# flash4242/Promptable-Counterfactual-GAN

Hardware: AMD Instinct MI355X
Metric: images/sec (G+D step) MNIST-28 cDCGAN bs512 @1/2/4/8 MI355X; % MFMA roofline (higher is better)
Workload: dtype f32

## Files before the change

include/pcgan_hip.h:

```cpp
#ifndef PCGAN_HIP_H
#define PCGAN_HIP_H

#include <stddef.h>
#include <stdint.h>

#ifdef __cplusplus
extern "C" {
#endif

typedef void* pcg_stream_t;

typedef enum pcg_status {
  PCG_OK = 0,
  PCG_ERR_INVALID = -1,
  PCG_ERR_WORKSPACE = -2,
  PCG_ERR_LAUNCH = -3,
  PCG_ERR_UNSUPPORTED = -4
} pcg_status;

typedef enum pcg_act {
  PCG_ACT_NONE = 0,
  PCG_ACT_RELU = 1,
  PCG_ACT_LRELU = 2,
  PCG_ACT_TANH = 3,
// ... 49 lines not shown
                         int64_t* num_batches_tracked, const float* gamma, const float* beta, float* coef_out ,
                         void* workspace, size_t workspace_bytes, pcg_stream_t stream);
int pcg_conv2d_dgrad_bn_xf(const pcg_conv_geom* g, const float* dy, const pcg_in_xform* xf, const float* w, const float* bias_x, float* dx,
                           float eps, float momentum, float* save_mean, float* save_invstd, float* running_mean, float* running_var,
                           int64_t* num_batches_tracked, const float* gamma, const float* beta, float* coef_out ,
                           void* workspace, size_t workspace_bytes, pcg_stream_t stream);
int pcg_conv2d_fwd_xf(const pcg_conv_geom* g, const float* x, const pcg_in_xform* xf, const float* w, const float* bias, int act,
                      float slope, float* y, void* workspace , size_t workspace_bytes, pcg_stream_t stream);
int pcg_conv2d_dgrad_xf(const pcg_conv_geom* g, const float* dy, const pcg_in_xform* xf, const float* w, const float* bias_x, int act,
                        float slope, float* dx, void* workspace , size_t workspace_bytes, pcg_stream_t stream);
int pcg_conv2d_wgrad_xf(const pcg_conv_geom* g, const float* x, const pcg_in_xform* xf_x, const float* dy, const pcg_in_xform* xf_dy,
                        float* dw, int accumulate, void* workspace, size_t workspace_bytes, pcg_stream_t stream);
int pcg_conv2d_dgrad_mask(const pcg_conv_geom* g, const float* dy, const float* w, const float* a_below, int act, float slope,
                          float* dx, void* workspace , size_t workspace_bytes, pcg_stream_t stream);
int32_t pcg_conv2d_dgrad_mask_thin_ok(const pcg_conv_geom* g);
int32_t pcg_conv2d_xf_thin_ok(const pcg_conv_geom* g);
int pcg_conv2d_fwd_add_mask(const pcg_conv_geom* g, const float* x, const float* w, const float* addend, const float* a_below, int act,
                            float slope, float* y, pcg_stream_t stream);
int pcg_conv2d_dgrad_add_mask(const pcg_conv_geom* g, const float* dy, const float* w, const float* addend, const float* a_below, int act,
                              float slope, float* dx, pcg_stream_t stream);
int pcg_conv2d_fwd_mask(const pcg_conv_geom* g, const float* x, const float* w, const float* a_below, int act, float slope,
                        float* y, void* workspace , size_t workspace_bytes, pcg_stream_t stream);
int pcg_conv2d_dgrad_bnbwd(const pcg_conv_geom* g, const float* dy, const float* w, const float* z_below, const float* mean,
                           const float* invstd, const float* gamma, const float* beta, int act, float slope, float* dx,
                           void* partial, size_t partial_bytes, pcg_stream_t stream);
int pcg_conv2d_fwd_bnbwd(const pcg_conv_geom* g, const float* x, const float* w, const float* z_below, const float* mean,
                         const float* invstd, const float* gamma, const float* beta, int act, float slope, float* y,
                         void* partial, size_t partial_bytes, pcg_stream_t stream);
int pcg_conv2d_dgrad_add(const pcg_conv_geom* g, const float* dy, const float* w, const float* addend, float* dx,
                         void* workspace , size_t workspace_bytes, pcg_stream_t stream);
// ... 440 lines not shown
```

promptable-counterfactual-gan_amd/_lib.py:

```python
import ctypes
import os

import torch

_HERE = os.path.dirname(os.path.abspath(__file__))
LIB_PATH = os.environ.get("PCG_LIB") or os.path.join(_HERE, "libpcgan_hip.so")

PCG_OK = 0
ACT_NONE, ACT_RELU, ACT_LRELU, ACT_TANH, ACT_SIGMOID = 0, 1, 2, 3, 4


class PcgError(RuntimeError):
    pass


class ConvGeom(ctypes.Structure):

    _fields_ = [(n, ctypes.c_int32) for n in ("B", "IH", "IW", "Cin", "OH", "OW", "Cout", "KH", "KW", "stride", "pad")]

    def key(self):
        return tuple(getattr(self, n) for n, _ in self._fields_)


_I, _P = ctypes.c_int32, ctypes.c_void_p
# ... 95 lines not shown
    "pcg_calib_mfma_workspace_bytes": (_sz, [_i32]),
    "pcg_calib_mfma": (_i, [_i32, _i32, _vp, _sz, _c.POINTER(_d), _c.POINTER(_c.c_uint64), _vp]),
    "pcg_calib_copy": (_i, [_vp, _vp, _i64, _vp]),
    "pcg_conv2d_fwd_workspace_bytes": (_sz, [_gp]),
    "pcg_conv2d_dgrad_workspace_bytes": (_sz, [_gp]),
    "pcg_conv2d_fwd": (_i, [_gp, _vp, _vp, _vp, _vp, _vp, _sz, _vp]),
    "pcg_conv2d_dgrad": (_i, [_gp, _vp, _vp, _vp, _vp, _vp, _sz, _vp]),
    "pcg_conv2d_fwd_act": (_i, [_gp, _vp, _vp, _vp, _i, _f, _vp, _vp, _sz, _vp]),
    "pcg_conv2d_dgrad_act": (_i, [_gp, _vp, _vp, _vp, _i, _f, _vp, _vp, _sz, _vp]),
    "pcg_conv2d_fwd_bn_workspace_bytes": (_sz, [_gp]),
    "pcg_conv2d_dgrad_bn_workspace_bytes": (_sz, [_gp]),
    "pcg_conv2d_fwd_bn": (_i, [_gp, _vp, _vp, _vp, _vp, _f, _f, _vp, _vp, _vp, _vp, _vp, _vp, _sz, _vp]),
    "pcg_conv2d_dgrad_bn": (_i, [_gp, _vp, _vp, _vp, _vp, _f, _f, _vp, _vp, _vp, _vp, _vp, _vp, _sz, _vp]),
    "pcg_conv2d_dgrad_mask": (_i, [_gp, _vp, _vp, _vp, _i, _f, _vp, _vp, _sz, _vp]),
    "pcg_conv2d_dgrad_mask_thin_ok": (_i32, [_gp]),
    "pcg_conv2d_xf_thin_ok": (_i32, [_gp]),
    "pcg_conv2d_fwd_add_mask": (_i, [_gp, _vp, _vp, _vp, _vp, _i, _f, _vp, _vp]),
    "pcg_conv2d_dgrad_add_mask": (_i, [_gp, _vp, _vp, _vp, _vp, _i, _f, _vp, _vp]),
    "pcg_conv2d_fwd_mask": (_i, [_gp, _vp, _vp, _vp, _i, _f, _vp, _vp, _sz, _vp]),
    "pcg_conv2d_dgrad_bnbwd": (_i, [_gp, _vp, _vp, _vp, _vp, _vp, _vp, _vp, _i, _f, _vp, _vp, _sz, _vp]),
    "pcg_conv2d_fwd_bnbwd": (_i, [_gp, _vp, _vp, _vp, _vp, _vp, _vp, _vp, _i, _f, _vp, _vp, _sz, _vp]),
    "pcg_conv2d_dgrad_add": (_i, [_gp, _vp, _vp, _vp, _vp, _vp, _sz, _vp]),
    "pcg_conv2d_fwd_bn_partial_rows": (_c.c_int32, [_gp]),
    "pcg_conv2d_dgrad_bn_partial_rows": (_c.c_int32, [_gp]),
    "pcg_bn_bwd_partial_workspace_bytes": (_sz, [_c.c_int32]),
    "pcg_bn_bwd_partial": (_i, [_vp, _vp, _i64, _c.c_int32, _vp, _vp, _vp, _vp, _c.c_int32, _vp, _vp, _vp, _i, _vp, _sz, _vp]),
    "pcg_conv2d_fwd_bn_xf": (_i, [_gp, _vp, _xp, _vp, _vp, _vp, _f, _f, _vp, _vp, _vp, _vp, _vp, _vp, _vp, _vp, _vp, _sz, _vp]),
    "pcg_conv2d_dgrad_bn_xf": (_i, [_gp, _vp, _xp, _vp, _vp, _vp, _f, _f, _vp, _vp, _vp, _vp, _vp, _vp, _vp, _vp, _vp, _sz, _vp]),
    "pcg_conv2d_fwd_xf": (_i, [_gp, _vp, _xp, _vp, _vp, _i, _f, _vp, _vp, _sz, _vp]),
    "pcg_conv2d_dgrad_xf": (_i, [_gp, _vp, _xp, _vp, _vp, _i, _f, _vp, _vp, _sz, _vp]),
# ... 177 lines not shown
```

promptable-counterfactual-gan_amd/csrc/conv_igemm.hip:

```cpp
#include <string.h>
#include <mutex>
#include "conv_loaders.h"
#include "thin_conv.h"

namespace pcg {
namespace {

__device__ __forceinline__ int wave_id() { return __builtin_amdgcn_readfirstlane((int)(threadIdx.x >> 6)); }

__device__ __forceinline__ void prio_entry(const ConvP& p) { if (p.edge_prio & 1) __builtin_amdgcn_s_setprio(3); }
__device__ __forceinline__ void prio_epilogue(const ConvP& p) { if (p.edge_prio & 2) __builtin_amdgcn_s_setprio(3); }

__device__ __forceinline__ int epi_group_off(const ConvP& p, int m_block) {
  return p.epi.group_rows > 0 ? __builtin_amdgcn_readfirstlane(m_block / p.epi.group_rows) * p.N : 0;
}

template <class Cfg, bool XF>
__global__ void __launch_bounds__(IG_THREADS, Cfg::MINW) conv_fwd_kernel(ConvP p) {
  extern __shared__ __attribute__((aligned(16))) float smem[];
  prio_entry(p);
  const uint32_t tile = xcd_remap(blockIdx.x, gridDim.x);
  const int mt = tile / p.tilesN, nt = tile % p.tilesN;
  const int m_block = mt * Cfg::BM, n_block = nt * Cfg::BN;
  const int kt_begin = blockIdx.y * p.ktiles_per_split;
// ... 59 lines not shown
    }
    DgradALoader<Cfg::BM, XF> la(p, f, m_block, tid);
    DgradBLoader<Cfg::BN> lb(p, f, n_block, tid);
    igemm_produce<Cfg>(la, lb, ktiles, smem, tid, ClockStamp{p.stamps, p.stamp_slots});
    return;
  }
  f32x16 acc[Cfg::TM][Cfg::TN];
  ClockStamp cs{p.stamps, p.stamp_slots};
  cs.phase(0);
  igemm_consume<Cfg, true, false>(ktiles, acc, smem, cs);
  prio_epilogue(p);
  igemm_store_tile<Cfg>(acc, smem, n_block, p.N, p.bias, [&](int row) -> float* {
    const int pix = rowpix[row];
    return pix >= 0 ? p.out + (size_t)pix * p.Cin + n_block : nullptr;
  }, p.stat_partial ? p.stat_partial + (size_t)(f.prow0 + mt * Cfg::WAVES_M) * 2 * p.N : nullptr, p.act, p.slope, &p.epi, epi_group_off(p, m_block));
  cs.phase(3);
}

struct SkPlan {
  int dp_tiles, sk_tiles, sk_blocks, ktiles;
  float* parts;
  int* arrivals;
};
struct SkSeg { int tile, kt_begin, nkt, nparts, first_block; };

__device__ __forceinline__ int sk_start(int g, const SkPlan& sk) {
  return __builtin_amdgcn_readfirstlane((int)((uint32_t)g * (uint32_t)(sk.sk_tiles * sk.ktiles) / (uint32_t)sk.sk_blocks));
}
__device__ __forceinline__ int sk_owner(int x, const SkPlan& sk) {
  return __builtin_amdgcn_readfirstlane((int)((((uint32_t)x + 1u) * (uint32_t)sk.sk_blocks - 1u) / (uint32_t)(sk.sk_tiles * sk.ktiles)));
// ... 981 lines not shown

extern "C" int32_t pcg_conv2d_xf_thin_ok(const pcg_conv_geom* g) { return check_geom(g) == PCG_OK && thin_conv_xf_ok(g) ? 1 : 0; }
extern "C" int32_t pcg_conv2d_dgrad_mask_thin_ok(const pcg_conv_geom* g) { return check_geom(g) == PCG_OK && thin_conv_dgrad_mask_ok(g) && g->Cin % 4 == 0 ? 1 : 0; }
extern "C" int pcg_conv2d_dgrad_mask(const pcg_conv_geom* g, const float* dy, const float* w, const float* a_below, int act, float slope,
                                     float* dx, void* workspace, size_t workspace_bytes, pcg_stream_t stream) {
  EpiAux e{};
  e.mode = EPI_MASK;
  if (int rc = check_geom(g)) return rc;
  if (pcg_conv2d_dgrad_mask_thin_ok(g)) {
    PCG_REQUIRE(dy && w && a_below && dx && (((uintptr_t)a_below | (uintptr_t)dx) & 15) == 0, "pcg_conv2d_dgrad_mask: null or misaligned tensor");
    PCG_REQUIRE(act == PCG_ACT_NONE || act == PCG_ACT_RELU || act == PCG_ACT_LRELU, "pcg_conv2d_dgrad_mask: activation %d is not none / ReLU / LeakyReLU", act);
    return thin_conv_dgrad_mask(g, dy, w, a_below, act, slope, dx, (hipStream_t)stream);
  }
  if (int rc = epi_common("pcg_conv2d_dgrad_mask", g, dx, a_below, act, slope, &e)) return rc;
  return conv2d_dgrad_impl(g, dy, w, nullptr, dx, nullptr, workspace, workspace_bytes, stream, PCG_ACT_NONE, 0.f, &e);
}
extern "C" int pcg_conv2d_fwd_mask(const pcg_conv_geom* g, const float* x, const float* w, const float* a_below, int act, float slope,
                                   float* y, void* workspace, size_t workspace_bytes, pcg_stream_t stream) {
  EpiAux e{};
  e.mode = EPI_MASK;
  if (int rc = check_geom(g)) return rc;
  if (int rc = epi_common("pcg_conv2d_fwd_mask", g, y, a_below, act, slope, &e)) return rc;
  return conv2d_fwd_impl(g, x, w, nullptr, y, nullptr, workspace, workspace_bytes, stream, PCG_ACT_NONE, 0.f, &e);
}

extern "C" int pcg_conv2d_dgrad_add(const pcg_conv_geom* g, const float* dy, const float* w, const float* addend, float* dx,
                                    void* workspace, size_t workspace_bytes, pcg_stream_t stream) {
  EpiAux e{};
  e.mode = EPI_ADD;
  if (int rc = check_geom(g)) return rc;
// ... 437 lines not shown
```

promptable-counterfactual-gan_amd/csrc/igemm_core.h:

```cpp
#pragma once
#include "pcg_common.h"

namespace pcg {

typedef float f32x16 __attribute__((ext_vector_type(16)));

typedef unsigned int u32x4 __attribute__((ext_vector_type(4)));
using rsrc_t = __amdgpu_buffer_rsrc_t;
constexpr uint32_t OOB_OFF = 0x80000000u;

__device__ __forceinline__ rsrc_t make_rsrc(const void* p, uint32_t bytes) {
  return __builtin_amdgcn_make_buffer_rsrc(const_cast<void*>(p), 0, bytes, 0x00020000);
}
__device__ __forceinline__ float4 buf_load4(rsrc_t r, uint32_t off) {
  const u32x4 v = __builtin_amdgcn_raw_buffer_load_b128(r, off, 0, 0);
  return make_float4(__uint_as_float(v.x), __uint_as_float(v.y), __uint_as_float(v.z), __uint_as_float(v.w));
}

constexpr int IG_LOADERS = 256;
constexpr int IG_THREADS = 512;
constexpr int IG_BK = 32;
#ifndef PCG_PREFETCH_DEPTH
#define PCG_PREFETCH_DEPTH 2
#endif
// ... 506 lines not shown
  }
  if (want_sums) {
#pragma unroll
    for (int off = Q; off < 64; off <<= 1) {
#pragma unroll
      for (int e = 0; e < 4; ++e) { s1[e] += __shfl_xor(s1[e], off); s2[e] += __shfl_xor(s2[e], off); }
    }
    if (r0 == 0 && nok) {
      double* pr = stat_row + (size_t)wm * 2 * N;
#pragma unroll
      for (int e = 0; e < 4; ++e) { pr[n + e] = s1[e]; pr[N + n + e] = s2[e]; }
    }
  }
}


}
```

promptable-counterfactual-gan_amd/csrc/thin_conv.h:

```cpp
#pragma once
#include "pcg_common.h"

namespace pcg {

inline bool thin_is_cin(const pcg_conv_geom* g) { return g->Cin <= 3; }
inline bool thin_is_cout(const pcg_conv_geom* g) { return g->Cout <= 3 && !thin_is_cin(g); }

struct ThinBnIn { const float* mean; const float* invstd; const float* gamma; const float* beta; int act; float slope; int groups; };
bool thin_conv_bnin_full_ok(const pcg_conv_geom* g, int groups);
int thin_conv_fwd(const pcg_conv_geom* g, const float* x, const float* w, const float* bias, float* y, void* ws,
                  size_t ws_bytes, hipStream_t s, int act = PCG_ACT_NONE, float slope = 0.f, const ThinBnIn* bnin = nullptr);
struct ThinXf { const float* scale; const float* shift; float neg; };
bool thin_conv_xf_ok(const pcg_conv_geom* g);
int thin_conv_dgrad(const pcg_conv_geom* g, const float* dy, const float* w, const float* bias_x, float* dx, void* ws,
                    size_t ws_bytes, hipStream_t s, int act = PCG_ACT_NONE, float slope = 0.f, const ThinXf* xf = nullptr);
size_t thin_conv_fwd_workspace_bytes(const pcg_conv_geom* g);
size_t thin_conv_dgrad_workspace_bytes(const pcg_conv_geom* g);
size_t thin_conv_wgrad_workspace_bytes(const pcg_conv_geom* g);
int thin_conv_wgrad(const pcg_conv_geom* g, const float* x, const float* dy, float* dw, int accumulate, void* ws,
                    size_t ws_bytes, hipStream_t s, const ThinXf* xf = nullptr, const ThinBnIn* bnin = nullptr);

bool thin_conv_fwd_bnbwd_ok(const pcg_conv_geom* g);
size_t thin_conv_fwd_bnbwd_workspace_bytes(const pcg_conv_geom* g);
int thin_conv_fwd_bnbwd(const pcg_conv_geom* g, const float* x, const float* w, const float* z, const float* mean, const float* invstd,
                        const float* gamma, const float* beta, int act, float slope, float* dz, float* dgamma, float* dbeta, int accumulate,
                        void* ws, size_t ws_bytes, hipStream_t s);

bool thin_conv_dgrad_mask_ok(const pcg_conv_geom* g);
int thin_conv_dgrad_mask(const pcg_conv_geom* g, const float* dy, const float* w, const float* a_below, int act, float slope, float* dx,
                         hipStream_t s);

bool thin_conv_dgrad_bnbwd_full_ok(const pcg_conv_geom* g, int groups);
size_t thin_conv_dgrad_bnbwd_full_workspace_bytes(const pcg_conv_geom* g, int groups);
int thin_conv_dgrad_bnbwd_full(const pcg_conv_geom* g, const float* dy, const float* w, const float* z, const float* mean, const float* invstd,
                               const float* gamma, const float* beta, int act, float slope, float* dz, float* dgamma, float* dbeta, int accumulate,
                               int groups, void* ws, size_t ws_bytes, hipStream_t s);

int launch_slab_reduce(const float* slab, float* dw, size_t n, size_t slab_stride, int nslabs, int accumulate, hipStream_t s, bool deferrable = false);

int slab_defer_begin(hipStream_t s);
int slab_defer_flush(hipStream_t s);
int slab_defer_pending();

}
```

promptable-counterfactual-gan_amd/csrc/thin_conv.hip:

```cpp
#include "thin_conv.h"
#include <cstdlib>

namespace pcg {
namespace {

struct ThinP {
  const float* thin;
  const float* wide;
  const float* w;
  const float* bias;
  float* out;
  int act; float slope;
  const float* xf_scale; const float* xf_shift; float xf_neg;
  const float* mask_src; float mask_neg;
  int B, TH, TW, Cs, WH, WW, C;
  int KH, KW, stride, pad, transposed;
  int wsS, wsT, wsC;
  int IH_, IW_;
  int QH, QW;
  int npix;
  FastDiv dIW, dIH, dCQ;
};

__device__ __forceinline__ bool tap_map(const ThinP& p, int ph, int pw, int kh, int kw, int& qh, int& qw) {
// ... 748 lines not shown
    }
    unsigned blocks = (unsigned)((n4 + 63) / 64);
    if (blocks > 4096) blocks = 4096;
    if (blocks == 0) blocks = 1;
    hipLaunchKernelGGL(slab_reduce4_kernel, dim3(blocks), dim3(64), 0, s, reinterpret_cast<const float4*>(slab),
                       reinterpret_cast<float4*>(dw), n4, slab_stride / 4, nslabs, accumulate);
  } else {
    unsigned blocks = (unsigned)((n + 255) / 256);
    if (blocks > 2048) blocks = 2048;
    if (blocks == 0) blocks = 1;
    hipLaunchKernelGGL(slab_reduce1_kernel, dim3(blocks), dim3(256), 0, s, slab, dw, n, slab_stride, nslabs, accumulate);
  }
  return launch_status("slab_reduce_kernel");
}

bool thin_conv_bnin_full_ok(const pcg_conv_geom* g, int groups) {
  if (!full_window(g) || groups < 1 || groups > 8 || g->B % groups || g->Cin % 4) return false;
  const int CQ = g->Cin / 4;
  return CQ <= 256 && 256 % CQ == 0 && (g->B / groups) % FULL_ROWS_DW == 0;
}
static FullXf full_xf_of(const pcg_conv_geom* g, const ThinBnIn* bi) {
  if (!bi || !bi->mean) return FullXf{nullptr, nullptr, nullptr, nullptr, 1.f, g->Cin, g->B};
  return FullXf{bi->mean, bi->invstd, bi->gamma, bi->beta, act_neg_of(bi->act, bi->slope), g->Cin, g->B / bi->groups};
}

int thin_conv_fwd(const pcg_conv_geom* g, const float* x, const float* w, const float* bias, float* y, void* ws,
                  size_t ws_bytes, hipStream_t s, int act, float slope, const ThinBnIn* bnin) {
  PCG_REQUIRE(!(bnin && bnin->mean) || (thin_conv_bnin_full_ok(g, bnin->groups) && (((uintptr_t)x | (uintptr_t)w) & 15) == 0),
              "thin conv forward: a BatchNorm input needs the full-window form (thin_conv_bnin_full_ok) and 16-byte aligned tensors");
  ThinP p{};
// ... 86 lines not shown
  if (cin_thin) { p.wide = dy; return launch_reduce(p, ws, ws_bytes, s); }
  p.thin = dy;
  const bool fuse = act_is_cheap(act);
  p.act = fuse ? act : PCG_ACT_NONE; p.slope = act_neg_of(p.act, slope);
  if (full_window(g) && bias_x == nullptr && (((uintptr_t)dx | (uintptr_t)w) & 15) == 0) {
    const int L4 = g->KH * g->KW * g->Cin / 4;
    hipLaunchKernelGGL(thin_full_outer_kernel, dim3((unsigned)((L4 + 255) / 256), (unsigned)((g->B + FULL_ROWS_DX - 1) / FULL_ROWS_DX)), dim3(256), 0, s, dy,
                       reinterpret_cast<const float4*>(w), reinterpret_cast<float4*>(dx), g->B, L4, p.slope);
    if (int e = launch_status("thin_full_outer_kernel")) return e;
    return fuse ? PCG_OK : pcg_act_fwd(dx, (int64_t)g->B * g->IH * g->IW * g->Cin, act, slope, dx, (pcg_stream_t)s);
  }
  if (int e = launch_expand(p, s)) return e;
  return fuse ? PCG_OK : pcg_act_fwd(dx, (int64_t)g->B * g->IH * g->IW * g->Cin, act, slope, dx, (pcg_stream_t)s);
}

bool thin_conv_dgrad_mask_ok(const pcg_conv_geom* g) {
  if (!thin_is_cout(g)) return false;
  ThinP p{};
  if (fill_common(p, g, false, false) != PCG_OK) return false;
  const bool k44 = p.KH == 4 && p.KW == 4, k33 = p.KH == 3 && p.KW == 3;
  RowsP rp{};
  size_t patch_bytes = 0;
  return (k44 || k33) && (k33 || p.Cs == 1) && lds_weight_bytes(p) <= 64 * 1024 && rows_plan(p, rp, &patch_bytes);
}
int thin_conv_dgrad_mask(const pcg_conv_geom* g, const float* dy, const float* w, const float* a_below, int act, float slope, float* dx,
                         hipStream_t s) {
  PCG_REQUIRE(thin_conv_dgrad_mask_ok(g), "thin grad-input with mask: only the row-block forms (k3 / k4 with a thin output)");
  ThinP p{};
  if (int e = fill_common(p, g, false, false)) return e;
  p.w = w; p.bias = nullptr; p.out = dx; p.thin = dy; p.act = PCG_ACT_NONE; p.slope = 0.f;
// ... 180 lines not shown
```

promptable-counterfactual-gan_amd/nn.py:

```python
import contextlib
import functools
import os

import torch
import torch.nn as nn

from . import ops
from ._lib import ACT_LRELU, ACT_NONE, ACT_RELU, ACT_SIGMOID, ACT_TANH, PcgError


def _pad4(n):
    return (n + 3) // 4 * 4


def in_conv_precision(fn):
    @functools.wraps(fn)
    def run(self, *args, **kwargs):
        with ops.conv_precision(self.conv_precision):
            return fn(self, *args, **kwargs)
    return run


class FlatModule(nn.Module):

# ... 536 lines not shown
                    else:
                        ops.conv2d_wgrad(g, a, dz, gw, acc, xf_x=xf_in)
                    if c.bias is not None and c.bias.requires_grad:
                        gb, accb = self._grad_view(c.bias)
                        ops.colsum(dz.numel() // C, C, dz, gb, accb)
                if defer is not None:
                    defer.join()
                if defer is not None and idx > 0 and g.Cin > 3 and g.Cout > 3:
                    defer.submit(wgrad_job, (dz, a))
                else:
                    wgrad_job()
            elif defer is not None:
                defer.join()
            if idx == 0:
                return None
            lo = self._blocks[idx - 1]
            _, _, zl, ml, il, yl, lo_eval, _ = saved[idx - 1]
            w = _w_ohwi(c.weight.data)
            fused = None
            mfma = g.Cin > 3 and g.Cout > 3 and g.Cin % 4 == 0 and g.Cout % 4 == 0 and g.stride <= 2
            if self.fuse_backward_epilogue and mfma and lo.act in (ACT_NONE, ACT_RELU, ACT_LRELU):
                if lo.bn is not None and not lo_eval and zl is not None and ops.group_dgrad_ok(g, G):
                    d, partial, nparts, nphases = ops.conv_bwd_data_fused_g(g, dz, w, lo.act, lo.slope, zl,
                                                                            (ml, il, lo.bn.weight.data, lo.bn.bias.data), G)
                    fused = ("bn", partial, nparts, nphases)
                    continue
                if lo.bn is None and lo.act != ACT_NONE:
                    res = ops.conv_bwd_data_fused(g, dz, w, False, lo.act, lo.slope, a_below=yl)
                    if res is not None:
                        d, fused = res[0], ("mask",)
                        continue
            if (self.fuse_backward_epilogue and lo.bn is not None and lo.act in (ACT_NONE, ACT_RELU, ACT_LRELU) and not lo_eval and zl is not None
                    and lo.bn.weight.requires_grad and self.fuse_full_window_bn and ops.full_dgrad_bn_bwd_ok(g, G)):
                dgl, accl = self._grad_view(lo.bn.weight)
                dbl, _ = self._grad_view(lo.bn.bias)
                d = ops.full_dgrad_bn_bwd(g, dz, w, zl, ml, il, lo.bn.weight.data, lo.bn.bias.data, lo.act, lo.slope, dgl, dbl, accl, groups=G)
                fused = ("done",)
                continue
            d = ops.conv2d_dgrad(g, dz, w)

    defer_slab_reductions = False

    fuse_full_window_bn = True

    wgrad_stream = None

    wgrad_overlap = None

    def _defer(self):
        if self.wgrad_overlap != "bn":
            return None
        side = self.__dict__.get("_overlap_stream")
        if side is None:
            side = self.__dict__["_overlap_stream"] = torch.cuda.Stream()
        return _WgradDefer(side, torch.cuda.current_stream())

# ... 65 lines not shown
                        ops.colsum(dz.numel() // C, C, dz, gb, accb)
                mfma = g.Cin > 3 and g.Cout > 3
                if defer is not None and mfma and idx > 0:
                    defer.join()
                    defer.submit(wgrad_job, (dz, a))
                else:
                    if defer is not None:
                        defer.join()
                    with torch.cuda.stream(side) if side is not None else contextlib.nullcontext():
                        wgrad_job()
            elif defer is not None:
                defer.join()
            last = idx == 0
            if last and not need_x:
                return None
            fused = None
            if not last and self.fuse_backward_epilogue:
                lo = self._blocks[idx - 1]
                _, _, zl, ml, il, yl, lo_eval, _ = saved[idx - 1]
                w = _w_ohwi(c.weight.data)
                res = None
                if lo.act in (ACT_NONE, ACT_RELU, ACT_LRELU) and not (b.transposed and b.flat):
                    if lo.bn is not None and not lo_eval and zl is not None:
                        res = ops.conv_bwd_data_fused(g, dz, w, b.transposed, lo.act, lo.slope, z_below=zl,
                                                      bn=(ml, il, lo.bn.weight.data, lo.bn.bias.data))
                        if res is not None:
                            d, fused = res[0], ("bn", res[1], res[2])
                    elif lo.bn is None and lo.act != ACT_NONE:
                        res = ops.conv_bwd_data_fused(g, dz, w, b.transposed, lo.act, lo.slope, a_below=yl)
                        if res is not None:
# ... 318 lines not shown
```

promptable-counterfactual-gan_amd/ops.py:

```python
import ctypes
import threading

import torch

from . import _lib
from ._lib import ACT_LRELU, ACT_NONE, ACT_RELU, ACT_SIGMOID, ACT_TANH, ConvGeom, check

_ws_cache = {}

_conv_hook = None


def set_conv_hook(hook):
    global _conv_hook
    _conv_hook = hook


def _conv_label(g, op):
    if g.Cin <= 3 or g.Cout <= 3:
        return f"thin_{op}"
    if op == "wgrad":
        n = g.KH * g.KW * g.Cin
        if g.Cout <= 64:
            return "conv_wgrad192_kernel<64x192>" if (n % 192 == 0 and n % 128 != 0) else "conv_wgrad_kernel<64x128>"
# ... 272 lines not shown
                  "pcg_conv2d_*_mask")
        return out, None, 0
    _chk(z_below, "z_below")
    assert z_below.numel() == out.numel()
    mean, invstd, gamma, beta = bn
    need = (lib.pcg_conv2d_fwd_bn_workspace_bytes if transposed else lib.pcg_conv2d_dgrad_bn_workspace_bytes)(ctypes.byref(g))
    if need == 0:
        return None
    nparts = (lib.pcg_conv2d_fwd_bn_partial_rows if transposed else lib.pcg_conv2d_dgrad_bn_partial_rows)(ctypes.byref(g))
    partial = torch.empty(need // 4, dtype=torch.float32, device=d.device)
    fn = lib.pcg_conv2d_fwd_bnbwd if transposed else lib.pcg_conv2d_dgrad_bnbwd
    with _Timed(g, "fwd" if transposed else "dgrad"):
        check(fn(ctypes.byref(g), _p(d), _p(w), _p(z_below), _p(mean), _p(invstd), _p(gamma), _p(beta), int(below_act), float(below_slope),
                 _p(out), _p(partial), need, _stream()), "pcg_conv2d_*_bnbwd")
    return out, partial, nparts


def conv_weight_adjoint(w):
    _chk(w, "w")
    Cout, KH, KW, Cin = w.shape
    wa = torch.empty((Cin, KH, KW, Cout), dtype=torch.float32, device=w.device)
    check(_lib.load().pcg_conv_weight_adjoint(_p(w), _p(wa), Cout, KH, KW, Cin, _stream()), "pcg_conv_weight_adjoint")
    return wa


def conv_weight_adjoint_many(ws):
    n = len(ws)
    Cout, KH, KW, Cin = ws[0].shape
    for w in ws:
        _chk(w, "w")
# ... 1097 lines not shown
```

Measured before the change: 51130.

## Fuse the thin first-layer backward tail into the second layer's dgrad kernel

Adds a dgrad kernel variant for the second discriminator conv whose epilogue applies the activation mask and then directly does the thin (Cin=1) first layer's work. One mode computes per-pixel tap products for grad-input followed by a col2im pass, enabled by default. The other accumulates weight-gradient partials into slots followed by a slot reduce, off by default. The aim is to avoid writing and re-reading the 64-channel gradient tensor and to save separate launches. The cost is more epilogue work and LDS use in the dgrad kernel, plus new workspace buffers.

```diff
diff --git a/include/pcgan_hip.h b/include/pcgan_hip.h
--- a/include/pcgan_hip.h
+++ b/include/pcgan_hip.h
@@ -87,6 +87,19 @@
 int pcg_conv2d_dgrad_mask(const pcg_conv_geom* g, const float* dy, const float* w, const float* a_below, int act, float slope,
                           float* dx, void* workspace , size_t workspace_bytes, pcg_stream_t stream);
 int32_t pcg_conv2d_dgrad_mask_thin_ok(const pcg_conv_geom* g);
+int32_t pcg_conv2d_dgrad_mask_wgrad_thin_ok(const pcg_conv_geom* g, const pcg_conv_geom* g0, int32_t groups);
+int32_t pcg_conv2d_dgrad_mask_taps_thin_ok(const pcg_conv_geom* g, const pcg_conv_geom* g0);
+size_t pcg_conv2d_dgrad_mask_taps_thin_workspace_bytes(const pcg_conv_geom* g0);
+int pcg_conv2d_dgrad_mask_taps_thin(const pcg_conv_geom* g, const float* dy, const float* w, const float* a_below, int act, float slope,
+                                    const pcg_conv_geom* g0, const float* w0, float* dx0, void* workspace, size_t workspace_bytes,
+                                    pcg_stream_t stream);
+size_t pcg_conv2d_dgrad_mask_wgrad_thin_workspace_bytes(const pcg_conv_geom* g);
+int pcg_conv2d_dgrad_mask_wgrad_thin(const pcg_conv_geom* g, const float* dy, const float* w, const float* a_below, int act, float slope,
+                                     const pcg_conv_geom* g0, const float* x0, float* dw0, int accumulate, void* workspace,
+                                     size_t workspace_bytes, pcg_stream_t stream);
+int pcg_conv2d_dgrad_mask_wgrad_thin_g(const pcg_conv_geom* g, const float* dy, const float* w, const float* a_below, int act, float slope,
+                                       const pcg_conv_geom* g0, const float* const* xs, int32_t groups, float* dw0, int accumulate,
+                                       void* workspace, size_t workspace_bytes, pcg_stream_t stream);
 int32_t pcg_conv2d_xf_thin_ok(const pcg_conv_geom* g);
 int pcg_conv2d_fwd_add_mask(const pcg_conv_geom* g, const float* x, const float* w, const float* addend, const float* a_below, int act,
                             float slope, float* y, pcg_stream_t stream);
diff --git a/promptable-counterfactual-gan_amd/_lib.py b/promptable-counterfactual-gan_amd/_lib.py
--- a/promptable-counterfactual-gan_amd/_lib.py
+++ b/promptable-counterfactual-gan_amd/_lib.py
@@ -133,6 +133,13 @@
     "pcg_conv2d_dgrad_bn": (_i, [_gp, _vp, _vp, _vp, _vp, _f, _f, _vp, _vp, _vp, _vp, _vp, _vp, _sz, _vp]),
     "pcg_conv2d_dgrad_mask": (_i, [_gp, _vp, _vp, _vp, _i, _f, _vp, _vp, _sz, _vp]),
     "pcg_conv2d_dgrad_mask_thin_ok": (_i32, [_gp]),
+    "pcg_conv2d_dgrad_mask_wgrad_thin_ok": (_i32, [_gp, _gp, _i32]),
+    "pcg_conv2d_dgrad_mask_wgrad_thin_workspace_bytes": (_sz, [_gp]),
+    "pcg_conv2d_dgrad_mask_wgrad_thin": (_i, [_gp, _vp, _vp, _vp, _i, _f, _gp, _vp, _vp, _i, _vp, _sz, _vp]),
+    "pcg_conv2d_dgrad_mask_wgrad_thin_g": (_i, [_gp, _vp, _vp, _vp, _i, _f, _gp, _vp, _i32, _vp, _i, _vp, _sz, _vp]),
+    "pcg_conv2d_dgrad_mask_taps_thin_ok": (_i32, [_gp, _gp]),
+    "pcg_conv2d_dgrad_mask_taps_thin_workspace_bytes": (_sz, [_gp]),
+    "pcg_conv2d_dgrad_mask_taps_thin": (_i, [_gp, _vp, _vp, _vp, _i, _f, _gp, _vp, _vp, _vp, _sz, _vp]),
     "pcg_conv2d_xf_thin_ok": (_i32, [_gp]),
     "pcg_conv2d_fwd_add_mask": (_i, [_gp, _vp, _vp, _vp, _vp, _i, _f, _vp, _vp]),
     "pcg_conv2d_dgrad_add_mask": (_i, [_gp, _vp, _vp, _vp, _vp, _i, _f, _vp, _vp]),
diff --git a/promptable-counterfactual-gan_amd/csrc/conv_igemm.hip b/promptable-counterfactual-gan_amd/csrc/conv_igemm.hip
--- a/promptable-counterfactual-gan_amd/csrc/conv_igemm.hip
+++ b/promptable-counterfactual-gan_amd/csrc/conv_igemm.hip
@@ -97,6 +97,51 @@
     const int pix = rowpix[row];
     return pix >= 0 ? p.out + (size_t)pix * p.Cin + n_block : nullptr;
   }, p.stat_partial ? p.stat_partial + (size_t)(f.prow0 + mt * Cfg::WAVES_M) * 2 * p.N : nullptr, p.act, p.slope, &p.epi, epi_group_off(p, m_block));
+  cs.phase(3);
+}
+
+template <class Cfg, bool TAPS>
+__global__ void __launch_bounds__(IG_THREADS, Cfg::MINW) conv_dgrad_thin_tail_kernel(ConvP p, DgradPhases phases, ThinTail tail) {
+  extern __shared__ __attribute__((aligned(16))) float smem[];
+  __shared__ int rowpix[Cfg::BM];
+  prio_entry(p);
+  uint32_t bx = blockIdx.x, py = blockIdx.y;
+  if (phases.interleave) {
+    const uint32_t l = xcd_remap(blockIdx.x, gridDim.x);
+    py = l % (uint32_t)phases.interleave; bx = l / (uint32_t)phases.interleave;
+  }
+  const PhaseInfo& f = phases.p[py];
+  const int tilesM = (f.Mp + Cfg::BM - 1) / Cfg::BM;
+  const uint32_t ntiles = (uint32_t)tilesM * p.tilesN;
+  if (bx >= ntiles) return;
+  const uint32_t tile = phases.interleave ? bx : xcd_remap(bx, ntiles);
+  const int m_block = (int)tile * Cfg::BM;
+  const int ktiles = f.nth * f.ntw * ((p.Cout + IG_BK - 1) / IG_BK);
+
+  if (wave_id() >= 4) {
+    const int tid = threadIdx.x - IG_LOADERS;
+    for (int r = tid; r < Cfg::BM; r += IG_LOADERS) {
+      const int m = m_block + r;
+      int pix = -1;
+      if (m < f.Mp) {
+        uint32_t t, cc, b, aa;
+        f.dPHw.divmod((uint32_t)m, t, cc);
+        f.dPHh.divmod(t, b, aa);
+        pix = ((int)b * p.IH + (int)aa * p.stride + f.ph) * p.IW + (int)cc * p.stride + f.pw;
+      }
+      rowpix[r] = pix;
+    }
+    DgradALoader<Cfg::BM, false> la(p, f, m_block, tid);
+    DgradBLoader<Cfg::BN> lb(p, f, 0, tid);
+    igemm_produce<Cfg>(la, lb, ktiles, smem, tid, ClockStamp{p.stamps, p.stamp_slots});
+    return;
+  }
+  f32x16 acc[Cfg::TM][Cfg::TN];
+  ClockStamp cs{p.stamps, p.stamp_slots};
+  cs.phase(0);
+  igemm_consume<Cfg, true, false>(ktiles, acc, smem, cs);
+  prio_epilogue(p);
+  igemm_thin_tail_tile<Cfg, TAPS>(acc, smem, rowpix, p.out, p.epi.neg, tail, (int)py * tilesM + (int)tile);
   cs.phase(3);
 }
 
@@ -1108,6 +1153,127 @@
   }
   if (int rc = epi_common("pcg_conv2d_dgrad_mask", g, dx, a_below, act, slope, &e)) return rc;
   return conv2d_dgrad_impl(g, dy, w, nullptr, dx, nullptr, workspace, workspace_bytes, stream, PCG_ACT_NONE, 0.f, &e);
+}
+
+constexpr int THIN_TAIL_MAX_GROUPS = 4;
+constexpr int THIN_TAIL_RED_ROWS = 32;
+static int thin_tail_slots(const pcg_conv_geom* g) {
+  DgradPhases ph{};
+  int maxMp = 0;
+  const int nph = build_phases(g, &ph, &maxMp);
+  return nph * ceil_div(maxMp, 128);
+}
+static bool thin_tail_geoms_ok(const pcg_conv_geom* g, const pcg_conv_geom* g0) {
+  if (!g || !g0 || check_geom(g) != PCG_OK || check_geom(g0) != PCG_OK || !mfma_layer(g) || conv_bf16()) return false;
+  if (g->Cin != 64 || g->Cout % 4 || g->stride != 2 || g->IH % 2 || g->IW % 2) return false;
+  return g0->Cin == 1 && g0->Cout == g->Cin && g0->KH == 4 && g0->KW == 4 && g0->B == g->B && g0->OH == g->IH && g0->OW == g->IW;
+}
+extern "C" int32_t pcg_conv2d_dgrad_mask_wgrad_thin_ok(const pcg_conv_geom* g, const pcg_conv_geom* g0, int32_t groups) {
+  if (!thin_tail_geoms_ok(g, g0)) return 0;
+  if (groups < 1 || groups > THIN_TAIL_MAX_GROUPS || g->B % groups) return 0;
+  return (int64_t)thin_tail_slots(g) * 64 * TAIL_TAPS * 4 < (1ll << 31) ? 1 : 0;
+}
+extern "C" size_t pcg_conv2d_dgrad_mask_wgrad_thin_workspace_bytes(const pcg_conv_geom* g) {
+  if (check_geom(g) != PCG_OK) return 0;
+  return ((size_t)thin_tail_slots(g) + THIN_TAIL_RED_ROWS) * 64 * TAIL_TAPS * sizeof(float);
+}
+template <class Cfg, bool TAPS>
+static int launch_dgrad_thin_tail(ConvP p, const DgradPhases& ph, int nphases, int maxMp, const ThinTail& tail, hipStream_t s) {
+  p.tilesN = 1;
+  const int tilesM = ceil_div(maxMp, Cfg::BM);
+  constexpr size_t smem_main = smem_bytes<Cfg, true, false>();
+  constexpr size_t smem_tail = sizeof(float) * (size_t)thin_tail_smem_floats<Cfg, TAPS>();
+  static_assert(smem_tail <= smem_main, "the thin tail fits the main loop's LDS: the workgroups per CU stay what they were");
+  static int once = set_smem(conv_dgrad_thin_tail_kernel<Cfg, TAPS>, smem_main);
+  if (once != PCG_OK) return once;
+  static const int il_env0 = getenv("PCG_DGRAD_INTERLEAVE") ? atoi(getenv("PCG_DGRAD_INTERLEAVE")) : 1;
+  const int il_env = g_tune.dgrad_interleave >= 0 ? g_tune.dgrad_interleave : il_env0;
+  DgradPhases phl = ph;
+  phl.interleave = (nphases > 1 && il_env && p.w_bytes <= (1u << 20)) ? nphases : 0;
+  if (phl.interleave)
+    hipLaunchKernelGGL((conv_dgrad_thin_tail_kernel<Cfg, TAPS>), dim3((unsigned)tilesM * nphases), dim3(IG_THREADS), smem_main, s, p, phl, tail);
+  else
+    hipLaunchKernelGGL((conv_dgrad_thin_tail_kernel<Cfg, TAPS>), dim3((unsigned)tilesM, nphases), dim3(IG_THREADS), smem_main, s, p, phl, tail);
+  return launch_status("conv_dgrad_thin_tail_kernel");
+}
+template <bool TAPS>
+static int launch_thin_tail(const ConvP& p, const DgradPhases& ph, int nphases, int maxMp, const ThinTail& tail, hipStream_t s) {
+  return g_tune.dgrad_swz3 == 0 ? launch_dgrad_thin_tail<Cfg128x64P, TAPS>(p, ph, nphases, maxMp, tail, s)
+                                : launch_dgrad_thin_tail<Cfg128x64, TAPS>(p, ph, nphases, maxMp, tail, s);
+}
+static int thin_tail_params(const char* who, const pcg_conv_geom* g, const float* dy, const float* w, const float* a_below, int act, float slope,
+                            ConvP* pp, DgradPhases* ph, int* maxMp) {
+  PCG_REQUIRE(dy && w && a_below, "%s: null pointer", who);
+  PCG_REQUIRE(act == PCG_ACT_NONE || act == PCG_ACT_RELU || act == PCG_ACT_LRELU, "%s: activation %d is not none / ReLU / LeakyReLU", who, act);
+  PCG_REQUIRE((((uintptr_t)a_below) & 15) == 0, "%s: tensors must be 16-byte aligned", who);
+  ConvP& p = *pp;
+  p = make_params(g);
+  p.dy = dy; p.w = w; p.out = const_cast<float*>(a_below);
+  p.epi.mode = EPI_MASK; p.epi.neg = act_neg_of(act, slope);
+  p.N = g->Cin;
+  const int nph = build_phases(g, ph, maxMp);
+  PCG_REQUIRE(nph == 4, "%s: empty phase", who);
+  return PCG_OK;
+}
+static int dgrad_mask_wgrad_thin(const char* who, const pcg_conv_geom* g, const float* dy, const float* w, const float* a_below, int act,
+                                 float slope, const pcg_conv_geom* g0, const float* const* xs, int groups, float* dw0, int accumulate,
+                                 void* workspace, size_t workspace_bytes, pcg_stream_t stream) {
+  PCG_REQUIRE(pcg_conv2d_dgrad_mask_wgrad_thin_ok(g, g0, groups), "%s: geometry not served (pcg_conv2d_dgrad_mask_wgrad_thin_ok)", who);
+  PCG_REQUIRE(dw0 && xs, "%s: null pointer", who);
+  for (int i = 0; i < groups; ++i) PCG_REQUIRE(xs[i] != nullptr, "%s: null input of group %d", who, i);
+  PCG_REQUIRE((((uintptr_t)dw0 | (uintptr_t)workspace) & 15) == 0, "%s: tensors must be 16-byte aligned", who);
+  const size_t need = pcg_conv2d_dgrad_mask_wgrad_thin_workspace_bytes(g);
+  if (!workspace || workspace_bytes < need) { set_error("%s: workspace %zu B < required %zu B", who, workspace_bytes, need); return PCG_ERR_WORKSPACE; }
+  ConvP p{};
+  DgradPhases ph{};
+  int maxMp = 0;
+  if (int e = thin_tail_params(who, g, dy, w, a_below, act, slope, &p, &ph, &maxMp)) return e;
+  float* slots = (float*)workspace;
+  const int nslots = thin_tail_slots(g);
+  ThinTail tail{xs[0], groups > 1 ? xs[1] : nullptr, groups > 2 ? xs[2] : nullptr, groups > 3 ? xs[3] : nullptr, g->B / groups,
+                g0->IH, g0->IW, g0->stride, g0->pad, g0->OH * g0->OW, g0->OW, slots, nullptr, nullptr, 0u};
+  hipStream_t st = (hipStream_t)stream;
+  if (int e = launch_thin_tail<false>(p, ph, 4, maxMp, tail, st)) return e;
+  return launch_slot_reduce(slots, dw0, (size_t)64 * TAIL_TAPS, nslots, slots + (size_t)nslots * 64 * TAIL_TAPS, THIN_TAIL_RED_ROWS, accumulate, st);
+}
+extern "C" int pcg_conv2d_dgrad_mask_wgrad_thin(const pcg_conv_geom* g, const float* dy, const float* w, const float* a_below, int act, float slope,
+                                                const pcg_conv_geom* g0, const float* x0, float* dw0, int accumulate, void* workspace,
+                                                size_t workspace_bytes, pcg_stream_t stream) {
+  const float* xs[1] = {x0};
+  return dgrad_mask_wgrad_thin("pcg_conv2d_dgrad_mask_wgrad_thin", g, dy, w, a_below, act, slope, g0, xs, 1, dw0, accumulate, workspace,
+                               workspace_bytes, stream);
+}
+extern "C" int pcg_conv2d_dgrad_mask_wgrad_thin_g(const pcg_conv_geom* g, const float* dy, const float* w, const float* a_below, int act,
+                                                  float slope, const pcg_conv_geom* g0, const float* const* xs, int32_t groups, float* dw0,
+                                                  int accumulate, void* workspace, size_t workspace_bytes, pcg_stream_t stream) {
+  return dgrad_mask_wgrad_thin("pcg_conv2d_dgrad_mask_wgrad_thin_g", g, dy, w, a_below, act, slope, g0, xs, groups, dw0, accumulate, workspace,
+                               workspace_bytes, stream);
+}
+
+extern "C" int32_t pcg_conv2d_dgrad_mask_taps_thin_ok(const pcg_conv_geom* g, const pcg_conv_geom* g0) {
+  return thin_tail_geoms_ok(g, g0) && thin_conv_dgrad_taps_ok(g0) && (int64_t)g0->B * g0->OH * g0->OW * TAIL_TAPS * 4 < (1ll << 31) ? 1 : 0;
+}
+extern "C" size_t pcg_conv2d_dgrad_mask_taps_thin_workspace_bytes(const pcg_conv_geom* g0) {
+  return check_geom(g0) == PCG_OK ? thin_conv_dgrad_taps_bytes(g0) : 0;
+}
+extern "C" int pcg_conv2d_dgrad_mask_taps_thin(const pcg_conv_geom* g, const float* dy, const float* w, const float* a_below, int act, float slope,
+                                               const pcg_conv_geom* g0, const float* w0, float* dx0, void* workspace, size_t workspace_bytes,
+                                               pcg_stream_t stream) {
+  const char* who = "pcg_conv2d_dgrad_mask_taps_thin";
+  PCG_REQUIRE(pcg_conv2d_dgrad_mask_taps_thin_ok(g, g0), "%s: geometry not served (pcg_conv2d_dgrad_mask_taps_thin_ok)", who);
+  PCG_REQUIRE(w0 && dx0, "%s: null pointer", who);
+  PCG_REQUIRE((((uintptr_t)workspace) & 15) == 0, "%s: workspace must be 16-byte aligned", who);
+  const size_t need = pcg_conv2d_dgrad_mask_taps_thin_workspace_bytes(g0);
+  if (!workspace || workspace_bytes < need) { set_error("%s: workspace %zu B < required %zu B", who, workspace_bytes, need); return PCG_ERR_WORKSPACE; }
+  ConvP p{};
+  DgradPhases ph{};
+  int maxMp = 0;
+  if (int e = thin_tail_params(who, g, dy, w, a_below, act, slope, &p, &ph, &maxMp)) return e;
+  ThinTail tail{};
+  tail.w0 = w0; tail.T = (float*)workspace; tail.plane = (uint32_t)(g0->B * g0->OH * g0->OW);
+  hipStream_t st = (hipStream_t)stream;
+  if (int e = launch_thin_tail<true>(p, ph, 4, maxMp, tail, st)) return e;
+  return thin_conv_dgrad_from_taps(g0, w0, (const float*)workspace, dx0, st);
 }
 extern "C" int pcg_conv2d_fwd_mask(const pcg_conv_geom* g, const float* x, const float* w, const float* a_below, int act, float slope,
                                    float* y, void* workspace, size_t workspace_bytes, pcg_stream_t stream) {
diff --git a/promptable-counterfactual-gan_amd/csrc/igemm_core.h b/promptable-counterfactual-gan_amd/csrc/igemm_core.h
--- a/promptable-counterfactual-gan_amd/csrc/igemm_core.h
+++ b/promptable-counterfactual-gan_amd/csrc/igemm_core.h
@@ -544,5 +544,114 @@
   }
 }
 
-
-}
+struct ThinTail {
+  const float* x0; const float* x1; const float* x2; const float* x3;
+  int group_imgs;
+  int H0, W0, stride0, pad0;
+  int OHW0, OW0;
+  float* slots;
+  const float* w0;
+  float* T;
+  uint32_t plane;
+};
+constexpr int TAIL_TAPS = 16;
+
+template <class Cfg, bool TAPS>
+constexpr int thin_tail_smem_floats() { return epilogue_smem_floats<Cfg>() + (TAPS ? 0 : Cfg::BM * TAIL_TAPS); }
+
+template <class Cfg, bool TAPS>
+__device__ __forceinline__ void igemm_thin_tail_tile(f32x16 (&acc)[Cfg::TM][Cfg::TN], float* smem, const int* rowpix, const float* a_below,
+                                                     float neg, const ThinTail& t, int slot) {
+  static_assert(Cfg::BM == 128 && Cfg::BN == 64 && Cfg::WAVES_M == 2 && Cfg::WAVES_N == 2, "the thin tail is written for 128x64 tiles");
+  constexpr int N = Cfg::BN, LDW = Cfg::WTN + 4, Q = Cfg::WTN / 4, RPI = 64 / Q, NK = Cfg::WTM / RPI, REG = Cfg::WTM * LDW;
+  const int lane = threadIdx.x & 63, wave = threadIdx.x >> 6;
+  const int wm = wave / Cfg::WAVES_N, wn = wave % Cfg::WAVES_N, li = lane & 31, lh = lane >> 5;
+  float* reg = smem + wave * REG;
+  float* Xs = smem + epilogue_smem_floats<Cfg>();
+#pragma unroll
+  for (int i = 0; i < Cfg::TM; ++i)
+#pragma unroll
+    for (int j = 0; j < Cfg::TN; ++j)
+#pragma unroll
+      for (int r = 0; r < 16; ++r) reg[(32 * i + acc_row(r, lh)) * LDW + 32 * j + li] = acc[i][j][r];
+  if constexpr (!TAPS) {
+    const int r = threadIdx.x >> 1, half = threadIdx.x & 1;
+    const int pix = rowpix[r];
+    float xv[8];
+#pragma unroll
+    for (int e = 0; e < 8; ++e) xv[e] = 0.f;
+    if (pix >= 0) {
+      const int b = pix / t.OHW0, rem = pix - b * t.OHW0, oh = rem / t.OW0, ow = rem - oh * t.OW0;
+      const int gi = b / t.group_imgs, bl = b - gi * t.group_imgs;
+      const float* xp = gi == 0 ? t.x0 : gi == 1 ? t.x1 : gi == 2 ? t.x2 : t.x3;
+      const int ih0 = oh * t.stride0 - t.pad0 + 2 * half, iw0 = ow * t.stride0 - t.pad0;
+#pragma unroll
+      for (int a = 0; a < 2; ++a)
+#pragma unroll
+        for (int c = 0; c < 4; ++c) {
+          const int ih = ih0 + a, iw = iw0 + c;
+          if (ih >= 0 && ih < t.H0 && iw >= 0 && iw < t.W0) xv[4 * a + c] = xp[((size_t)bl * t.H0 + ih) * t.W0 + iw];
+        }
+    }
+    *reinterpret_cast<float4*>(Xs + r * TAIL_TAPS + 8 * half) = make_float4(xv[0], xv[1], xv[2], xv[3]);
+    *reinterpret_cast<float4*>(Xs + r * TAIL_TAPS + 8 * half + 4) = make_float4(xv[4], xv[5], xv[6], xv[7]);
+  }
+  asm volatile("s_waitcnt lgkmcnt(0)" ::: "memory");
+  const int cq = lane % Q, r0 = lane / Q;
+  float4 u[NK];
+#pragma unroll
+  for (int k = 0; k < NK; ++k) {
+    const int pix = rowpix[wm * Cfg::WTM + r0 + RPI * k];
+    u[k] = pix >= 0 ? *reinterpret_cast<const float4*>(a_below + (size_t)pix * N + wn * Cfg::WTN + 4 * cq) : make_float4(0.f, 0.f, 0.f, 0.f);
+  }
+#pragma unroll
+  for (int k = 0; k < NK; ++k) {
+    const int row = r0 + RPI * k;
+    float4 v = *reinterpret_cast<const float4*>(reg + row * LDW + 4 * cq);
+    if (rowpix[wm * Cfg::WTM + row] < 0) v = make_float4(0.f, 0.f, 0.f, 0.f);
+    v.x *= u[k].x > 0.f ? 1.f : neg; v.y *= u[k].y > 0.f ? 1.f : neg; v.z *= u[k].z > 0.f ? 1.f : neg; v.w *= u[k].w > 0.f ? 1.f : neg;
+    *reinterpret_cast<float4*>(reg + row * LDW + 4 * cq) = v;
+  }
+  __syncthreads();
+  typedef float f32x4_t __attribute__((ext_vector_type(4)));
+  const int col = lane & 15, h = lane >> 4;
+  auto dz = [&](int q, int c) { return smem[((q / Cfg::WTM) * Cfg::WAVES_N + c / Cfg::WTN) * REG + (q % Cfg::WTM) * LDW + c % Cfg::WTN]; };
+  if constexpr (TAPS) {
+    float bw[4][4];
+#pragma unroll
+    for (int jj = 0; jj < 4; ++jj)
+#pragma unroll
+      for (int e = 0; e < 4; ++e) bw[jj][e] = t.w0[(16 * jj + 4 * h + e) * TAIL_TAPS + col];
+    const int qa = 32 * wave + col, qb = qa + 16;
+    f32x4_t accA = {0.f, 0.f, 0.f, 0.f}, accB = {0.f, 0.f, 0.f, 0.f};
+#pragma unroll
+    for (int jj = 0; jj < 4; ++jj)
+#pragma unroll
+      for (int e = 0; e < 4; ++e) {
+        accA = __builtin_amdgcn_mfma_f32_16x16x4f32(dz(qa, 16 * jj + 4 * h + e), bw[jj][e], accA, 0, 0, 0);
+        accB = __builtin_amdgcn_mfma_f32_16x16x4f32(dz(qb, 16 * jj + 4 * h + e), bw[jj][e], accB, 0, 0, 0);
+      }
+    float* plane = t.T + (size_t)col * t.plane;
+#pragma unroll
+    for (int r = 0; r < 4; ++r) {
+      const int pa = rowpix[32 * wave + 4 * h + r], pb = rowpix[32 * wave + 16 + 4 * h + r];
+      if (pa >= 0) plane[pa] = accA[r];
+      if (pb >= 0) plane[pb] = accB[r];
+    }
+  } else {
+    const int cb = 16 * wave;
+    f32x4_t p0 = {0.f, 0.f, 0.f, 0.f}, p1 = {0.f, 0.f, 0.f, 0.f};
+#pragma unroll
+    for (int ks = 0; ks < Cfg::BM / 4; ks += 2) {
+      const int q0 = 4 * ks + h, q1 = q0 + 4;
+      p0 = __builtin_amdgcn_mfma_f32_16x16x4f32(dz(q0, cb + col), Xs[q0 * TAIL_TAPS + col], p0, 0, 0, 0);
+      p1 = __builtin_amdgcn_mfma_f32_16x16x4f32(dz(q1, cb + col), Xs[q1 * TAIL_TAPS + col], p1, 0, 0, 0);
+    }
+    float* dst = t.slots + (size_t)slot * (N * TAIL_TAPS) + (cb + 4 * h) * TAIL_TAPS + col;
+#pragma unroll
+    for (int r = 0; r < 4; ++r) dst[r * TAIL_TAPS] = p0[r] + p1[r];
+  }
+}
+
+
+}
diff --git a/promptable-counterfactual-gan_amd/csrc/thin_conv.h b/promptable-counterfactual-gan_amd/csrc/thin_conv.h
--- a/promptable-counterfactual-gan_amd/csrc/thin_conv.h
+++ b/promptable-counterfactual-gan_amd/csrc/thin_conv.h
@@ -26,6 +26,10 @@
                         const float* gamma, const float* beta, int act, float slope, float* dz, float* dgamma, float* dbeta, int accumulate,
                         void* ws, size_t ws_bytes, hipStream_t s);
 
+bool thin_conv_dgrad_taps_ok(const pcg_conv_geom* g);
+size_t thin_conv_dgrad_taps_bytes(const pcg_conv_geom* g);
+int thin_conv_dgrad_from_taps(const pcg_conv_geom* g, const float* w, const float* T, float* dx, hipStream_t s);
+
 bool thin_conv_dgrad_mask_ok(const pcg_conv_geom* g);
 int thin_conv_dgrad_mask(const pcg_conv_geom* g, const float* dy, const float* w, const float* a_below, int act, float slope, float* dx,
                          hipStream_t s);
@@ -38,6 +42,8 @@
 
 int launch_slab_reduce(const float* slab, float* dw, size_t n, size_t slab_stride, int nslabs, int accumulate, hipStream_t s, bool deferrable = false);
 
+int launch_slot_reduce(const float* slots, float* dw, size_t n, int nslots, float* mid, int rows, int accumulate, hipStream_t s);
+
 int slab_defer_begin(hipStream_t s);
 int slab_defer_flush(hipStream_t s);
 int slab_defer_pending();
diff --git a/promptable-counterfactual-gan_amd/csrc/thin_conv.hip b/promptable-counterfactual-gan_amd/csrc/thin_conv.hip
--- a/promptable-counterfactual-gan_amd/csrc/thin_conv.hip
+++ b/promptable-counterfactual-gan_amd/csrc/thin_conv.hip
@@ -786,6 +786,24 @@
   return launch_status("slab_reduce_kernel");
 }
 
+int launch_slot_reduce(const float* slots, float* dw, size_t n, int nslots, float* mid, int rows, int accumulate, hipStream_t s) {
+  PCG_REQUIRE(n % 4 == 0 && (((uintptr_t)slots | (uintptr_t)dw | (uintptr_t)mid) & 15) == 0, "launch_slot_reduce: misaligned");
+  const size_t n4 = n / 4;
+  const float4* src = reinterpret_cast<const float4*>(slots);
+  int ns = nslots;
+  if (nslots >= 64 * rows && nslots % rows == 0) {
+    const size_t m4 = n4 * rows;
+    hipLaunchKernelGGL(slab_reduce4_wide_kernel, dim3((unsigned)((m4 + 15) / 16)), dim3(256), 0, s, src, reinterpret_cast<float4*>(mid), m4, m4,
+                       nslots / rows, 0);
+    if (int e = launch_status("slab_reduce4_wide_kernel")) return e;
+    src = reinterpret_cast<const float4*>(mid);
+    ns = rows;
+  }
+  hipLaunchKernelGGL(slab_reduce4_wide_kernel, dim3((unsigned)((n4 + 15) / 16)), dim3(256), 0, s, src, reinterpret_cast<float4*>(dw), n4, n4,
+                     ns, accumulate);
+  return launch_status("slab_reduce4_wide_kernel");
+}
+
 bool thin_conv_bnin_full_ok(const pcg_conv_geom* g, int groups) {
   if (!full_window(g) || groups < 1 || groups > 8 || g->B % groups || g->Cin % 4) return false;
   const int CQ = g->Cin / 4;
@@ -902,6 +920,36 @@
   return fuse ? PCG_OK : pcg_act_fwd(dx, (int64_t)g->B * g->IH * g->IW * g->Cin, act, slope, dx, (pcg_stream_t)s);
 }
 
+bool thin_conv_dgrad_taps_ok(const pcg_conv_geom* g) {
+  if (!thin_is_cin(g) || g->Cin != 1 || g->Cout != 64 || g->KH * g->KW > 16) return false;
+  ThinP p{};
+  if (fill_common(p, g, true, false) != PCG_OK) return false;
+  return !fast32_ok(p) && reduce_scratch_bytes(p) != 0 && lds_weight_bytes(p) <= 64 * 1024;
+}
+size_t thin_conv_dgrad_taps_bytes(const pcg_conv_geom* g) {
+  ThinP p{};
+  if (fill_common(p, g, true, false) != PCG_OK) return 0;
+  return reduce_scratch_bytes(p);
+}
+int thin_conv_dgrad_from_taps(const pcg_conv_geom* g, const float* w, const float* T, float* dx, hipStream_t s) {
+  PCG_REQUIRE(thin_conv_dgrad_taps_ok(g), "thin grad-input from tap products: geometry not served");
+  ThinP p{};
+  if (int e = fill_common(p, g, true, false)) return e;
+  p.act = PCG_ACT_NONE; p.w = w; p.out = dx;
+  const size_t need = reduce_scratch_bytes(p);
+  const uint32_t plane = (uint32_t)(p.B * p.WH * p.WW);
+  if (p.transposed && p.stride == 2 && p.KH == 4 && p.KW == 4 && p.IW_ % 4 == 0 && (((uintptr_t)p.out) & 15) == 0) {
+    unsigned b4 = (unsigned)((p.npix / 4 + 255) / 256);
+    if (b4 > 8192) b4 = 8192;
+    hipLaunchKernelGGL(thin_col2im_s2k4_kernel, dim3(b4), dim3(256), 0, s, p, T, (uint32_t)need, plane);
+    return launch_status("thin_col2im_s2k4_kernel");
+  }
+  unsigned b2 = (unsigned)((p.npix + 255) / 256);
+  if (b2 > 8192) b2 = 8192;
+  hipLaunchKernelGGL(thin_col2im_kernel, dim3(b2), dim3(256), 0, s, p, T, (uint32_t)need, plane);
+  return launch_status("thin_col2im_kernel");
+}
+
 bool thin_conv_dgrad_mask_ok(const pcg_conv_geom* g) {
   if (!thin_is_cout(g)) return false;
   ThinP p{};
diff --git a/promptable-counterfactual-gan_amd/nn.py b/promptable-counterfactual-gan_amd/nn.py
--- a/promptable-counterfactual-gan_amd/nn.py
+++ b/promptable-counterfactual-gan_amd/nn.py
@@ -574,6 +574,8 @@
                 defer.join()
             if idx == 0:
                 return None
+            if idx == 1 and self._thin_wgrad_tail(g, dz, c, saved[0], G):
+                return None
             lo = self._blocks[idx - 1]
             _, _, zl, ml, il, yl, lo_eval, _ = saved[idx - 1]
             w = _w_ohwi(c.weight.data)
@@ -600,6 +602,46 @@
             d = ops.conv2d_dgrad(g, dz, w)
 
     defer_slab_reductions = False
+
+    fuse_thin_taps_tail = os.environ.get("PCG_THIN_TAPS_TAIL", "1") != "0"
+    fuse_thin_wgrad_tail = os.environ.get("PCG_THIN_WGRAD_TAIL", "0") == "1"
+
+    def _thin_tail_geom(self, g, saved0):
+        if not self.fuse_backward_epilogue:
+            return None
+        b0, b1 = self._blocks[0], self._blocks[1]
+        c0 = b0.conv
+        g0, _, _, _, _, y0, eval0, xf0 = saved0
+        if (b0.transposed or b1.transposed or getattr(b0, "flat", False) or getattr(b1, "flat", False) or b0.bn is not None
+                or b0.act not in (ACT_RELU, ACT_LRELU) or (c0.bias is not None and c0.bias.requires_grad) or xf0 is not None or y0 is None
+                or eval0):
+            return None
+        return ops.conv_geom(g.B, g0.IH, g0.IW, g0.Cin, g0.Cout, g0.KH, g0.KW, g0.stride, g0.pad)
+
+    def _thin_taps_tail(self, g, dz, c, saved0):
+        if not self.fuse_thin_taps_tail:
+            return None
+        gf = self._thin_tail_geom(g, saved0)
+        if gf is None or not ops.dgrad_mask_taps_thin_ok(g, gf):
+            return None
+        b0 = self._blocks[0]
+        return ops.conv_dgrad_mask_taps_thin(g, dz, _w_ohwi(c.weight.data), saved0[5], b0.act, b0.slope, gf, _w_ohwi(b0.conv.weight.data))
+
+    def _thin_wgrad_tail(self, g, dz, c, saved0, G):
+        if not self.fuse_thin_wgrad_tail:
+            return False
+        gf = self._thin_tail_geom(g, saved0)
+        c0 = self._blocks[0].conv
+        if gf is None or not c0.weight.requires_grad or not ops.dgrad_mask_wgrad_thin_ok(g, gf, G):
+            return False
+        a0 = saved0[1]
+        xs = list(a0) if isinstance(a0, (list, tuple)) else [a0]
+        if len(xs) != G:
+            return False
+        b0 = self._blocks[0]
+        gw, acc = self._grad_view(c0.weight)
+        ops.conv_dgrad_mask_wgrad_thin(g, dz, _w_ohwi(c.weight.data), saved0[5], b0.act, b0.slope, gf, xs, _w_ohwi(gw), acc)
+        return True
 
     fuse_full_window_bn = True
 
@@ -695,6 +737,12 @@
             last = idx == 0
             if last and not need_x:
                 return None
+            if idx == 1 and not need_x and need_p and not b.transposed and self._thin_wgrad_tail(g, dz, c, saved[0], 1):
+                return None
+            if idx == 1 and need_x and not need_p and not b.transposed:
+                dx0 = self._thin_taps_tail(g, dz, c, saved[0])
+                if dx0 is not None:
+                    return dx0
             fused = None
             if not last and self.fuse_backward_epilogue:
                 lo = self._blocks[idx - 1]
diff --git a/promptable-counterfactual-gan_amd/ops.py b/promptable-counterfactual-gan_amd/ops.py
--- a/promptable-counterfactual-gan_amd/ops.py
+++ b/promptable-counterfactual-gan_amd/ops.py
@@ -310,6 +310,49 @@
         check(fn(ctypes.byref(g), _p(d), _p(w), _p(z_below), _p(mean), _p(invstd), _p(gamma), _p(beta), int(below_act), float(below_slope),
                  _p(out), _p(partial), need, _stream()), "pcg_conv2d_*_bnbwd")
     return out, partial, nparts
+
+
+def dgrad_mask_wgrad_thin_ok(g, g0, groups=1):
+    return bool(_lib.load().pcg_conv2d_dgrad_mask_wgrad_thin_ok(ctypes.byref(g), ctypes.byref(g0), int(groups)))
+
+
+def conv_dgrad_mask_wgrad_thin(g, d, w, a_below, below_act, below_slope, g0, xs, dw0, accumulate):
+    lib = _lib.load()
+    _chk(d, "d"); _chk(w, "w"); _chk(a_below, "a_below"); _chk(dw0, "dw0")
+    for x in xs:
+        _chk(x, "x")
+        assert x.numel() == (g0.B // len(xs)) * g0.IH * g0.IW
+    assert a_below.numel() == g.B * g.IH * g.IW * g.Cin and dw0.numel() == g0.Cout * g0.KH * g0.KW
+    need = lib.pcg_conv2d_dgrad_mask_wgrad_thin_workspace_bytes(ctypes.byref(g))
+    ws = workspace(need, d.device)
+    with _Timed(g, "dgrad"):
+        if len(xs) == 1:
+            check(lib.pcg_conv2d_dgrad_mask_wgrad_thin(ctypes.byref(g), _p(d), _p(w), _p(a_below), int(below_act), float(below_slope),
+                                                       ctypes.byref(g0), _p(xs[0]), _p(dw0), int(bool(accumulate)), _p(ws), ws.numel(), _stream()),
+                  "pcg_conv2d_dgrad_mask_wgrad_thin")
+        else:
+            ptrs = _ptr_array(xs)
+            check(lib.pcg_conv2d_dgrad_mask_wgrad_thin_g(ctypes.byref(g), _p(d), _p(w), _p(a_below), int(below_act), float(below_slope),
+                                                         ctypes.byref(g0), ptrs, len(xs), _p(dw0), int(bool(accumulate)), _p(ws), ws.numel(),
+                                                         _stream()), "pcg_conv2d_dgrad_mask_wgrad_thin_g")
+    return dw0
+
+
+def dgrad_mask_taps_thin_ok(g, g0):
+    return bool(_lib.load().pcg_conv2d_dgrad_mask_taps_thin_ok(ctypes.byref(g), ctypes.byref(g0)))
+
+
+def conv_dgrad_mask_taps_thin(g, d, w, a_below, below_act, below_slope, g0, w0):
+    lib = _lib.load()
+    _chk(d, "d"); _chk(w, "w"); _chk(a_below, "a_below"); _chk(w0, "w0")
+    assert a_below.numel() == g.B * g.IH * g.IW * g.Cin and w0.numel() == g0.Cout * g0.KH * g0.KW * g0.Cin
+    dx = torch.empty((g0.B, g0.IH, g0.IW, g0.Cin), dtype=torch.float32, device=d.device)
+    need = lib.pcg_conv2d_dgrad_mask_taps_thin_workspace_bytes(ctypes.byref(g0))
+    ws = workspace(need, d.device)
+    with _Timed(g, "dgrad"):
+        check(lib.pcg_conv2d_dgrad_mask_taps_thin(ctypes.byref(g), _p(d), _p(w), _p(a_below), int(below_act), float(below_slope), ctypes.byref(g0),
+                                                  _p(w0), _p(dx), _p(ws), ws.numel(), _stream()), "pcg_conv2d_dgrad_mask_taps_thin")
+    return dx
 
 
 def conv_weight_adjoint(w):
```

Result: no change. 51310, median of 6 (+0.4%).
